# xcmyz/FastVocoder

Measured on AMD Instinct MI355X. Metric: audio samples/sec + RTF @22.05kHz, HiFi-GAN-light, 1/2/4/8 MI355X, higher is better.
Workload: dtype f32 (products as split-f16 pairs, fp32 accumulate); 1 GPU; HiFi-GAN light (conf/hifigan/light.yaml) generator forward, mel 80x1000, batch 1 utterance(s) per GPU, 240000 samples each; BASELINE.json configs[1]; global_batch=1, frames=1000, parallelism=single GPU, plan_ops_per_forward=25

## Files before the change

### fastvocoder_amd/_native.py

```python
import ctypes
import os
import subprocess

import torch

_HERE = os.path.dirname(os.path.abspath(__file__))
LIB_PATH = os.path.join(_HERE, "libfastvocoder_hip.so")
_CSRC = os.path.join(_HERE, "csrc")
SOURCES = ["conv_mfma.hip", "api.hip", "plan.hip", "pack.hip", "pqmf.hip", "wav_sink.hip", "mel.hip", "resample.hip", "griffin_lim.hip", "stft_loss.hip", "stft_loss_grad.hip", "stft_mag_grad.hip", "disc.hip", "disc_grad.hip", "disc_wgrad.hip", "mpd.hip", "mpd_grad.hip", "mpd_wgrad.hip", "gen_grad.hip", "gen_grad_bf16.hip", "basis_grad.hip", "basis_learn.hip", "optim.hip", "conv_inst_narrow.hip",
           "pair_launch.hip", "pair_inst_c16.hip", "pair_inst_c32.hip", "pairh_inst_c16.hip", "pairh_inst_c32.hip",
           "convh_launch.hip", "convh_inst_c64.hip", "convh_inst_c128.hip", "convt_inst.hip",
           "convg_inst.hip", "convr_inst.hip", "convtn_inst.hip", "convk_inst.hip", "convq2_inst.hip",
           "mrfh_launch.hip", "mrfh_inst_a.hip", "mrfh_inst_b.hip", "mrfw_inst.hip", "convtl_inst.hip", "convs2_inst.hip", "convu2_inst.hip"] + \
          [f"conv_inst_s{i}.hip" for i in range(6)]
HEADERS = ["fv_internal.h", "launch_host.hpp", "conv_kernels.hpp", "pair_kernels.hpp", "pair_inst.hpp", "pairh_kernels.hpp",
           "pairh_inst.hpp", "convh_kernels.hpp", "convh_inst.hpp", "convr_kernels.hpp",
           "convtn_kernels.hpp", "convk_kernels.hpp", "convq2_kernels.hpp", "mrfh_kernels.hpp", "mrfh_inst.hpp", "mrfw_kernels.hpp", "convtl_kernels.hpp", "convs2_kernels.hpp", "convu2_kernels.hpp", "api_internal.h", "stft_core.hpp", "basis_grad_host.hpp", "wgrad_tile.hpp", "gen_grad_host.hpp"]

PAD_ZERO, PAD_REFLECT = 0, 1
PAD_CAUSAL = 2
POST_NONE, POST_TANH, POST_RELU = 0, 1, 2
SLOT_NONE, SLOT_IN, SLOT_OUT, SLOT_TMP0, MAX_SLOTS = -1, 0, 1, 2, 32
SLOT_AUX_IN0, SLOT_AUX_IN1, SLOT_OUT2 = 28, 29, 30
ABI_VERSION = 18
# ... 280 lines not shown
    L.fv_pack_pair_weight.argtypes = [vp, vp, i, i, vp]
    L.fv_resblock1_fused.argtypes = [i, pp, pp, pp, pp, pp, pp, pp, ctypes.POINTER(i), i, i, i, i, f, f, vp]
    L.fv_mrf_stage.argtypes = [pp, pp, pp, pp, pp, vp, vp, ctypes.POINTER(i), i, i, i, i, f, f, i, f, vp]
    L.fv_plan_add_resblock_pair.argtypes = [vp, i, i, i, vp, vp, vp, vp, i, i, i, f, f]
    L.fv_packed_pair_floats_ex.argtypes = [i, i, i]
    L.fv_packed_pair_floats_ex.restype = i64
    L.fv_pack_pair_weight_ex.argtypes = [vp, vp, i, i, i, vp, vp]
    L.fv_resblock1_fused_ex.argtypes = [i, pp, pp, pp, pp, pp, pp, pp, pp, pp, pp, ctypes.POINTER(i), i, i, i, i, f, f,
                                        i, f, i, vp, vp]
    L.fv_plan_add_resblock_pair_ex.argtypes = [vp, i, i, i, i, i, i, vp, vp, vp, vp, i, i, i, f, f, i, f, i]
    L.fv_conv1d_split_f16.argtypes = [i, pp, pp, pp, pp, pp, pp, pp, pp, ctypes.POINTER(i), i, i, i, i, i, f, f, i, f, vp, vp]
    L.fv_plan_set_pair_output_conv.argtypes = [vp, vp, vp, i, f, i]
    L.fv_packed_mrf_stage_floats.argtypes = [i, ctypes.POINTER(i)]
    L.fv_packed_mrf_stage_floats.restype = i64
    L.fv_pack_mrf_stage_split_f16.argtypes = [pp, pp, pp, pp, vp, i, ctypes.POINTER(i), vp, vp]
    L.fv_mrf_stage_workspace_bytes.argtypes = [i]
    L.fv_mrf_stage_workspace_bytes.restype = i64
    L.fv_mrf_stage_split_f16.argtypes = [vp, vp, vp, vp, i, i, i, ctypes.POINTER(i), ctypes.POINTER(i), f, f, i, f, vp, vp, vp,
                                         vp, i64, vp, vp]
    L.fv_plan_add_mrf_stage_split_f16.argtypes = [vp, i, i, i, vp, i, ctypes.POINTER(i), ctypes.POINTER(i), f, f, i, f, vp, i64]
    L.fv_plan_add_conv1d_split_f16.argtypes = [vp, i, i, i, i, i, i, vp, vp, i, i, i, i, f, f, i, f]
    L.fv_plan_add_mrf_sum.argtypes = [vp, ctypes.POINTER(i), i, i, pp, pp, pp, pp, i, ctypes.POINTER(i), i, f, f, i, f]
    L.fv_plan_create.argtypes = [i]
    L.fv_plan_create.restype = vp
    L.fv_plan_destroy.argtypes = [vp]
    L.fv_plan_destroy.restype = None
    L.fv_plan_add_conv1d.argtypes = [vp, i, i, i, i, i, i, vp, vp, i, i, i, i, i, i, f, f, i, f]
    L.fv_plan_add_conv_transpose1d.argtypes = [vp, i, i, i, vp, vp, i, i, i, i, i, i, f, i, f]
    L.fv_plan_add_pqmf_synthesis.argtypes = [vp, i, i, vp, i, i]
    L.fv_plan_set_guard.argtypes = [vp, vp]
    L.fv_plan_check_range.argtypes = [vp, vp]
    L.fv_tuning_set.argtypes = [ctypes.c_char_p, i]
    L.fv_debug_pair_schedule.argtypes = [i, ctypes.POINTER(i), ctypes.POINTER(i), i, i, i, ctypes.POINTER(ctypes.c_uint)]
    L.fv_debug_mrf_class_schedule.argtypes = [i, i, i, i, ctypes.POINTER(ctypes.c_int64), ctypes.POINTER(ctypes.c_uint)]
    L.fv_debug_mrf_stage_class_f16.argtypes = [vp, vp, vp, i, i, i, i, ctypes.POINTER(i), ctypes.POINTER(i), f, vp, i64, vp]
    L.fv_mrf_stage_classes_f16.argtypes = [vp, vp, vp, vp, i, i, i, ctypes.POINTER(i), ctypes.POINTER(i), f, vp, i64, vp, vp]
    L.fv_plan_add_mrf_stage_classes_f16.argtypes = [vp, i, i, i, vp, i, ctypes.POINTER(i), ctypes.POINTER(i), f, vp, i64]
    L.fv_plan_set_group.argtypes = [vp, i]
    L.fv_plan_output_shape.argtypes = [vp, i, ctypes.POINTER(i), ctypes.POINTER(i64)]
    L.fv_plan_workspace_bytes.argtypes = [vp, i, i]
    L.fv_plan_workspace_bytes.restype = i64
    L.fv_plan_run.argtypes = [vp, i, i, vp, vp, vp, i64, vp]
    L.fv_plan_run_aux.argtypes = [vp, i, i, vp, vp, vp, ctypes.POINTER(vp), ctypes.POINTER(i), vp, i64, vp]
    L.fv_plan_set_output_offset.argtypes = [vp, i, i]
    L.fv_plan_slot_shape.argtypes = [vp, i, i, ctypes.POINTER(i), ctypes.POINTER(i64)]
    L.fv_plan_num_ops.argtypes = [vp]
    L.fv_profile_enable.argtypes = [i]
    L.fv_profile_bracket_cost.argtypes = [vp, i, ctypes.POINTER(ctypes.c_double)]
    L.fv_profile_mfma_f16_rate.argtypes = [vp, i64, i, i, vp, ctypes.POINTER(ctypes.c_double)]
    L.fv_profile_collect.argtypes = [i, ctypes.POINTER(i64), ctypes.POINTER(ctypes.c_double),
                                     ctypes.POINTER(ctypes.c_double), ctypes.POINTER(ctypes.c_double)]
    if L.fv_version() != ABI_VERSION:
        raise NativeError(f"ABI mismatch: library reports {L.fv_version()}, binding expects {ABI_VERSION}")
    _lib = L
    return L


def check(rc):
    if rc != 0:
        raise NativeError(f"libfastvocoder_hip error {rc}: {lib().fv_last_error().decode()}")


def _ptr(t, name="tensor", allow_none=False):
    if t is None:
        if allow_none:
            return None
# ... 33 lines not shown
        self.t = torch.zeros(2, dtype=torch.int32).pin_memory()

    def ptr(self, i=0):
        return self.t.data_ptr() + 4 * i

    def peek(self, i=0):
        return int(self.t[i])

    def clear(self, i=0):
        self.t[i] = 0


def tuning_set(key, value):
    check(lib().fv_tuning_set(key.encode(), int(value)))


def debug_pair_schedule(n_items, cost, nblk, mode=0, three_members=False):
    n = len(n_items)
    arr = ctypes.c_int * n
    table = (ctypes.c_uint * 512)()
    rc = lib().fv_debug_pair_schedule(n, arr(*[int(v) for v in n_items]), arr(*[int(v) for v in cost]), int(nblk), int(mode),
                                      1 if three_members else 0, table)
    check(rc if rc < 0 else 0)
    if rc == 1:
        out = []
        for b in range(nblk):
            w0, w1 = table[2 * b], table[2 * b + 1]
            e = [w0 & 0xFFFF, w0 >> 16, w1 & 0xFFFF]
            out.append([(v & 2047, v >> 11) for v in e[:n]])
        return 1, out
    if rc == 2:
        return 2, [int(table[i]) for i in range(nblk)]
    return 0, None


def mrf_class_schedule(batch, t, nblk, force=False):
    info = (ctypes.c_int64 * 12)()
    table = (ctypes.c_uint * 512)()
    check(lib().fv_debug_mrf_class_schedule(int(batch), int(t), int(nblk), 1 if force else 0, info, table))
    keys = ("split", "n_a", "n_b", "makespan", "makespan_one", "reach_a", "reach_b", "window", "cost_a", "cost_b", "cost_one")
    out = {k: int(info[i]) for i, k in enumerate(keys)}
    out["split"] = bool(out["split"])
    out["ranges"] = [(int(table[2 * i]), int(table[2 * i + 1])) for i in range(out["n_a"] + out["n_b"])]
    return out


def _flag_ptr(flag):
    if flag is None:
        return None
    if isinstance(flag, GuardWord):
        return flag.ptr(1)
    if isinstance(flag, int):
        return flag
    return flag.data_ptr()


def _guard_ptr(guard):
    if guard is None:
        return None
    if isinstance(guard, GuardWord):
        return guard.ptr(0)
    return guard.data_ptr()



def fold_weight_norm(v, g):
# ... 1624 lines not shown
```

### fastvocoder_amd/csrc/api.hip

```cpp
#include <stdarg.h>
#include <stdio.h>
#include <stdlib.h>

#include <string>
#include <mutex>
#include <utility>
#include <vector>

#include <ctype.h>
#include <string.h>
#include <unistd.h>

#include "api_internal.h"
#include "launch_host.hpp"

namespace fv {

static thread_local std::string g_err;

int fail(int code, const char* fmt, ...) {
    char buf[512];
    va_list ap;
    va_start(ap, fmt);
    vsnprintf(buf, sizeof(buf), fmt, ap);
// ... 276 lines not shown
namespace fv {
int allow_dynamic_lds(const void* kernel, size_t bytes) {
    if (bytes <= 64 * 1024) return 0;
    struct Grant { const void* kernel; int device; size_t bytes; };
    static std::mutex mu;
    static std::vector<Grant> granted;
    int dev = 0;
    FV_HIP(hipGetDevice(&dev));
    std::lock_guard<std::mutex> lock(mu);
    for (Grant& g : granted)
        if (g.kernel == kernel && g.device == dev) {
            if (g.bytes >= bytes) return 0;
            FV_HIP(hipFuncSetAttribute(kernel, hipFuncAttributeMaxDynamicSharedMemorySize, (int)bytes));
            g.bytes = bytes;
            return 0;
        }
    FV_HIP(hipFuncSetAttribute(kernel, hipFuncAttributeMaxDynamicSharedMemorySize, (int)bytes));
    granted.push_back({kernel, dev, bytes});
    return 0;
}

static Tuning g_tuning;
static std::once_flag g_tuning_once;
struct TuningEntry {
    const char* key;
    int Tuning::*field;
};
static const TuningEntry kTuningTable[] = {
    {"pair_dbg", &Tuning::pair_dbg},       {"dbg", &Tuning::conv_dbg},           {"sched", &Tuning::sched},
    {"sched_switch", &Tuning::sched_switch}, {"convh_skel", &Tuning::convh_skel}, {"convp_skel", &Tuning::convp_skel},
    {"convq_skel", &Tuning::convq_skel},   {"pair128_unfused", &Tuning::pair128_unfused},
    {"convg_rows64", &Tuning::convg_rows64}, {"stack_items", &Tuning::stack_items}, {"stack_wide", &Tuning::stack_wide},
    {"convp_wide", &Tuning::convp_wide},   {"convq_wide", &Tuning::convq_wide},
    {"convh_rows64", &Tuning::convh_rows64},  {"convt_rows64", &Tuning::convt_rows64},
    {"pairh_skel", &Tuning::pairh_skel},   {"pair_skel", &Tuning::pair_skel},    {"convh_blocks", &Tuning::convh_blocks},
    {"pair_blocks", &Tuning::pair_blocks}, {"sum3_min", &Tuning::sum3_min},      {"lds_budget", &Tuning::lds_budget},
    {"units", &Tuning::units},             {"shape16", &Tuning::shape16},        {"shape32", &Tuning::shape32},
    {"shape64", &Tuning::shape64},         {"krows", &Tuning::krows},            {"grid_cap", &Tuning::grid_cap},
    {"no_group", &Tuning::no_group},       {"mrf_blocks", &Tuning::mrf_blocks},  {"mrf_shape", &Tuning::mrf_shape},
    {"mrf_prio", &Tuning::mrf_prio},       {"convt_lean", &Tuning::convt_lean},
    {"mrf_cost_a", &Tuning::mrf_cost_a},   {"mrf_cost_b", &Tuning::mrf_cost_b},  {"mrf_cost_one", &Tuning::mrf_cost_one},
    {"convs_ringfree", &Tuning::convs_ringfree}, {"convu_resident", &Tuning::convu_resident},
};
static void tuning_from_env() {
    const char* on = getenv("FV_TUNING");
    if (!on || atoi(on) != 1) return;
    for (const TuningEntry& e : kTuningTable) {
        char name[64] = "FV_";
        size_t n = 3;
        for (const char* c = e.key; *c && n + 1 < sizeof(name); ++c) name[n++] = (char)toupper((unsigned char)*c);
        name[n] = 0;
        const char* v = getenv(name);
        if (v && *v) g_tuning.*(e.field) = atoi(v);
    }
    const char* tp = getenv("FV_PAIR_TRACE_PTR");
    if (tp && *tp) g_tuning.trace_ptr = strtoull(tp, nullptr, 0);
}
const Tuning& tuning() {
    std::call_once(g_tuning_once, tuning_from_env);
    return g_tuning;
}

int device_cu_count() {
    static int cus = 0;
    if (!cus) {
        int dev = 0, v = 0;
// ... 885 lines not shown
        if (strcmp(e.key, key) == 0) {
            g_tuning.*(e.field) = value;
            return 0;
        }
    static const char* const kRetiredKeys[] = {"convp_pp"};
    for (const char* retired : kRetiredKeys)
        if (value == 0 && strcmp(retired, key) == 0) return 0;
    return fail(FV_ERR_INVALID_ARG, "tuning_set: unknown key '%s'", key);
}

int fv_debug_pair_schedule(int n_members, const int* n_items, const int* cost, int nblk, int mode, int three_members,
                           unsigned* table) {
    if (!n_items || !cost || !table) return fail(FV_ERR_INVALID_ARG, "debug_pair_schedule: null argument");
    if (n_members < 1 || n_members > 3) return fail(FV_ERR_INVALID_ARG, "debug_pair_schedule: %d members", n_members);
    if (mode != 0 && mode != 1) return fail(FV_ERR_INVALID_ARG, "debug_pair_schedule: mode %d", mode);
    if (nblk < 1 || nblk > (mode == 0 ? fv::kSchedBlocks : 2 * fv::kSchedBlocks))
        return fail(FV_ERR_INVALID_ARG, "debug_pair_schedule: %d blocks", nblk);
    fv::PairParams p = {};
    p.n_members = n_members;
    long long n[3] = {0, 0, 0};
    for (int m = 0; m < n_members; ++m) {
        if (n_items[m] < 0 || n_items[m] >= (1LL << 31) / nblk || cost[m] < 1 || cost[m] > 65535)
            return fail(FV_ERR_INVALID_ARG, "debug_pair_schedule: member %d", m);
        p.m[m].n_items = n_items[m];
        p.m[m].cost = cost[m];
        n[m] = n_items[m];
    }
    if (mode == 0) fv::pair_schedule(p, nblk, three_members != 0);
    else fv::pair_cut_schedule(p, nblk, n);
    memcpy(table, p.sched, sizeof(p.sched));
    return p.sched_on;
}

int fv_profile_enable(int on) {
    g_prof_on = on != 0;
    g_prof_need_start = true;
    return 0;
}

__global__ void profile_null_kernel() {}

int fv_profile_bracket_cost(void* stream, int n, double* ms_per_bracket) {
    if (n <= 0 || !ms_per_bracket) return fail(FV_ERR_INVALID_ARG, "profile_bracket_cost: n=%d", n);
    hipStream_t s = (hipStream_t)stream;
    ScopedEvents events((size_t)n + 4);
    if (int rc = events.create()) return rc;
    const std::vector<hipEvent_t>& ev = events.ev;
    for (int i = 0; i < 8; ++i) hipLaunchKernelGGL(profile_null_kernel, dim3(1), dim3(64), 0, s);
    FV_HIP(hipEventRecord(ev[n], s));
    for (int i = 0; i < n; ++i) {
        hipLaunchKernelGGL(profile_null_kernel, dim3(1), dim3(64), 0, s);
        FV_HIP(hipEventRecord(ev[i], s));
    }
    FV_HIP(hipEventRecord(ev[n + 1], s));
    for (int i = 0; i < n; ++i) hipLaunchKernelGGL(profile_null_kernel, dim3(1), dim3(64), 0, s);
    FV_HIP(hipEventRecord(ev[n + 2], s));
    FV_HIP(hipEventSynchronize(ev[n + 2]));
    float with = 0.f, without = 0.f;
    FV_HIP(hipEventElapsedTime(&with, ev[n], ev[n - 1]));
    FV_HIP(hipEventElapsedTime(&without, ev[n + 1], ev[n + 2]));
    const double cost = ((double)with - (double)without) / n;
    *ms_per_bracket = cost > 0 ? cost : 0;
    return 0;
}

typedef _Float16 peak_f16x8 __attribute__((ext_vector_type(8)));
// ... 76 lines not shown
```

### fastvocoder_amd/csrc/convh_launch.hip

```cpp
#include <stdlib.h>
#include <string.h>

#include <algorithm>
#include <array>
#include <map>
#include <mutex>
#include <vector>

#include "launch_host.hpp"

namespace fv {

extern template int launch_convh_geom<4, 2>(const PairParams&, int, size_t, hipStream_t);
extern template int launch_convh_geom<2, 2>(const PairParams&, int, size_t, hipStream_t);


void pair_schedule(PairParams& p, int nblk, bool three_members) {
    typedef std::array<unsigned, 2 * kSchedBlocks> Table;
    static std::mutex mu;
    static std::map<std::array<int, 9>, Table> cache;
    p.sched_on = 0;
    const Tuning& tn = tuning();
    if (tn.sched == 0) return;
    long long items = 0;
// ... 250 lines not shown
    if (p.B <= 0 || p.T <= 0) return 0;
    if (C != 128 && C != 256 && C != 512)
        return fail(FV_ERR_UNSUPPORTED, "split-f16 two-source 1x1 conv: C = %d (128, 256 or 512)", C);
    if (int rc = check_desc_range(fam, C, p.T)) return rc;
    if (int rc = check_slopes(fam, p.slope, p.act_slope)) return rc;
    PairMember& mb = p.m[0];
    if (int rc = check_tensors(fam, mb, -1, kNeedX2 | kNeedY)) return rc;
    if (int rc = check_aligned(fam, mb, 0)) return rc;
    p.n_members = 1;
    p.ctot = C;
    p.nch = 2 * C / 128;
    p.nmt = C / 64;
    p.reflect = 0;
    p.out_div = 1.f;
    const int NTC = 128;
    mb.k = 1;
    mb.n_tiles = (p.T + NTC - 1) / NTC;
    const bool wide = tuning().convg_rows64 < 0 ? (long long)mb.n_tiles * p.B * (p.nmt / 2) * 10 >= 7LL * device_cu_count()
                                                : !tuning().convg_rows64;
    mb.n_items = mb.n_tiles * p.B * (wide ? p.nmt / 2 : p.nmt);
    mb.cost = 1;
    LdsLayout lds;
    p.x_off = lds.add(4 * 16384 / 4);
    p.img_off = lds.add(4 * 128 * 128 / 4);
    p.nblk = (int)persistent_blocks(mb.n_items, 1, tuning().convh_blocks);
    p.sched_on = 0;
    set_debug(p);
    ProfileScope prof(s, FV_KERNEL_CONVG, Work{2.0 * p.B * (double)C * 2 * C * p.T,
                                               4.0 * (2.0 * C * C + (double)p.B * C * p.T * (3 + (mb.res ? 1 : 0) + (mb.y_act ? 1 : 0)))});
    return wide ? launch_convr_geom(p, lds.bytes(), s) : launch_convg_geom(p, lds.bytes(), s);
}

constexpr int kPair64Wide = 65, kPair128Wide = 129;
template <int DIL, int C>
int launch_convq2_dil(const PairParams& p, size_t lds, hipStream_t s);
extern template int launch_convq2_dil<1, 128>(const PairParams&, size_t, hipStream_t);
extern template int launch_convq2_dil<3, 128>(const PairParams&, size_t, hipStream_t);
extern template int launch_convq2_dil<5, 128>(const PairParams&, size_t, hipStream_t);
extern template int launch_convq2_dil<1, 64>(const PairParams&, size_t, hipStream_t);
extern template int launch_convq2_dil<3, 64>(const PairParams&, size_t, hipStream_t);
extern template int launch_convq2_dil<5, 64>(const PairParams&, size_t, hipStream_t);
extern template int launch_convq2_dil<1, kPair64Wide>(const PairParams&, size_t, hipStream_t);
extern template int launch_convq2_dil<3, kPair64Wide>(const PairParams&, size_t, hipStream_t);
extern template int launch_convq2_dil<5, kPair64Wide>(const PairParams&, size_t, hipStream_t);
extern template int launch_convq2_dil<1, kPair128Wide>(const PairParams&, size_t, hipStream_t);
extern template int launch_convq2_dil<3, kPair128Wide>(const PairParams&, size_t, hipStream_t);

#ifndef FV_WARM_TILES
#define FV_WARM_TILES 1
#endif
static void warm_run_costs(PairParams& p, long long items, int nm) {
    if (!FV_WARM_TILES || items < 8LL * p.nblk) return;
    for (int i = 0; i < p.n_members; ++i) p.m[i].cost *= nm - (p.m[i].k - 1);
}

struct FusedPair {
    int C;
    int narrow, wide;
    int Tuning::*wide_from;
    int wide_dil;
    int Tuning::*skel;
    int skel_auto;
    bool three_members;
    int kind;
};
static const FusedPair kFusedPair64 = {64, 128, 256, &Tuning::convp_wide, 5, &Tuning::convp_skel, 0, false, FV_KERNEL_CONVH64};
static const FusedPair kFusedPair128 = {128, 64, 128, &Tuning::convq_wide, 3, &Tuning::convq_skel, 5, true, FV_KERNEL_CONVH128};

static int launch_fused_pair(const FusedPair& f, PairParams& p, int dil, hipStream_t s) {
    const char* const fam = "resblock pair";
    const int C = f.C;
    if (p.B <= 0 || p.T <= 0) return 0;
    if (dil != 1 && dil != 3 && dil != 5) return fail(FV_ERR_UNSUPPORTED, "resblock pair: dilation %d (1, 3 or 5)", dil);
    if (int rc = check_launch(fam, p, C)) return rc;
    sort_members_by_taps(p);
    long long wide_items = 0;
    for (int i = 0; i < p.n_members; ++i) wide_items += (long long)p.B * ((p.T + f.wide - p.m[i].k) / (f.wide + 1 - p.m[i].k));
    const bool wide = dil <= f.wide_dil && wide_items * 10 >= (long long)(tuning().*f.wide_from) * device_cu_count();
    const int NM = wide ? f.wide : f.narrow;
    const int skel = f.skel_auto && tuning().*f.skel < 0 ? f.skel_auto : tuning().*f.skel;
    int img_bytes = 0;
    long long items = 0;
    for (int i = 0; i < p.n_members; ++i) {
        PairMember& mb = p.m[i];
        if (int rc = check_taps(fam, mb.k)) return rc;
        if (int rc = check_member(fam, mb, i, kNeedW2 | kNeedY)) return rc;
        const int nout = NM - (mb.k - 1);
        mb.n_tiles = (p.T + nout - 1) / nout;
        mb.n_items = mb.n_tiles * p.B;
        mb.cost = C / 32 * mb.k + skel;
        const int xrows = (NM + (mb.k - 1) * dil + 3) / 4 * 4;
        const int img = 4 * C * ((xrows + 15) / 16 * 16);
        if (img > img_bytes) img_bytes = img;
        items += mb.n_items;
    }
    LdsLayout lds;
    p.x_off = 0;
    p.img_off = lds.add((size_t)img_bytes / 4);
    p.mid_off = lds.add((size_t)4 * C * (NM + 16) / 4);
    p.bias_off = lds.add(4 * (size_t)C + 16);
    if (int rc = check_lds(fam, lds.bytes())) return rc;
    p.nblk = (int)persistent_blocks(items, 1, tuning().convh_blocks);
    pair_schedule(p, p.nblk, f.three_members);
    if (!p.sched_on) {
        warm_run_costs(p, items, NM);
        cut_table(p, p.nblk);
    }
    set_debug(p);
    ProfileScope prof(s, f.kind, pair_work(p, C));
    const size_t bytes = lds.bytes();
    if (C == 64)
        return wide ? by_dilation<1, 3, 5>(dil, [&](auto d) { return launch_convq2_dil<decltype(d)::value, kPair64Wide>(p, bytes, s); })
                    : by_dilation<1, 3, 5>(dil, [&](auto d) { return launch_convq2_dil<decltype(d)::value, 64>(p, bytes, s); });
    return wide ? by_dilation<1, 3, 3>(dil, [&](auto d) { return launch_convq2_dil<decltype(d)::value, kPair128Wide>(p, bytes, s); })
                : by_dilation<1, 3, 5>(dil, [&](auto d) { return launch_convq2_dil<decltype(d)::value, 128>(p, bytes, s); });
}

int launch_convp(PairParams p, int dil, hipStream_t s) { return launch_fused_pair(kFusedPair64, p, dil, s); }
int launch_convq(PairParams p, int dil, hipStream_t s) { return launch_fused_pair(kFusedPair128, p, dil, s); }

}
```

### fastvocoder_amd/csrc/convq2_inst.hip

```cpp
#include "convq2_kernels.hpp"
namespace fv {
template <int DIL, int C>
int launch_convq2_dil(const PairParams& p, size_t lds, hipStream_t s) {
    if (int rc = allow_dynamic_lds(reinterpret_cast<const void*>(convq2_kernel<DIL, C>), lds)) return rc;
    hipLaunchKernelGGL((convq2_kernel<DIL, C>), dim3(p.nblk), dim3(512), lds, s, p);
    FV_HIP(hipGetLastError());
    return 0;
}
template int launch_convq2_dil<1, 128>(const PairParams&, size_t, hipStream_t);
template int launch_convq2_dil<3, 128>(const PairParams&, size_t, hipStream_t);
template int launch_convq2_dil<5, 128>(const PairParams&, size_t, hipStream_t);
template int launch_convq2_dil<1, 64>(const PairParams&, size_t, hipStream_t);
template int launch_convq2_dil<3, 64>(const PairParams&, size_t, hipStream_t);
template int launch_convq2_dil<5, 64>(const PairParams&, size_t, hipStream_t);
template int launch_convq2_dil<1, kPair64Wide>(const PairParams&, size_t, hipStream_t);
template int launch_convq2_dil<3, kPair64Wide>(const PairParams&, size_t, hipStream_t);
template int launch_convq2_dil<5, kPair64Wide>(const PairParams&, size_t, hipStream_t);
template int launch_convq2_dil<1, kPair128Wide>(const PairParams&, size_t, hipStream_t);
template int launch_convq2_dil<3, kPair128Wide>(const PairParams&, size_t, hipStream_t);
}
```

### fastvocoder_amd/csrc/convq2_kernels.hpp

```cpp
#pragma once
#include "convh_kernels.hpp"
#ifndef FV_WARM_TILES
#define FV_WARM_TILES 1
#endif

namespace fv {

template <int KT_, int DIL_>
struct ConvQGeom {
    static constexpr int KT = KT_, DIL = DIL_, C = 128, CG = 4, CB = 16, NFW = 2, NT = 512;
    static constexpr int NM = 64;
    static constexpr int NOUT = NM - (KT - 1);
    static constexpr int P1 = (KT - 1) * DIL / 2, P2 = (KT - 1) / 2;
    static constexpr int NSTEP = KT * CG;
    static constexpr int NST = 2 * NSTEP;
    static constexpr int XROWS = (NM + (KT - 1) * DIL + 3) / 4 * 4;
    static constexpr int XRP = (XROWS + 15) / 16 * 16;
    static constexpr int XHALF = CB * XRP * 16;
    static constexpr int XR = (XROWS * CB + NT - 1) / NT, XRM = XR;
    static constexpr int MRP = NM + 16;
    static constexpr int MHALF = CB * MRP * 16;
    static constexpr int STAGE_BYTES = 16384, RING = 3, AHEAD = RING - 1;
    static constexpr int WTILE = NSTEP * 8192;
    static constexpr int RAWST = NST - 8;
#ifndef FV_CONVQ_BDEPTH
#define FV_CONVQ_BDEPTH 2
#endif
    static constexpr int BD = FV_CONVQ_BDEPTH;
    static constexpr int NRAW = XRM * 8;
    static_assert(KT - 1 <= 16 && NSTEP >= 8, "taps");
    static_assert(((CG - 1) * 4 * XRP + (KT - 1) * DIL + 16 * (NFW - 1)) * 16 + 16 < 65536, "ds_read immediate range");
};

template <int KT_, int DIL_>
struct ConvPGeom {
    typedef ConvHGeom<2, 2, KT_, DIL_> H;
    static constexpr int KT = KT_, DIL = DIL_, C = 64, NFW = 2;
    static constexpr int NM = H::NTC;
    static constexpr int NOUT = NM - (KT - 1);
    static constexpr int P1 = (KT - 1) * DIL / 2, P2 = (KT - 1) / 2;
    static constexpr int NST1 = H::NST, NST = 2 * NST1;
    static constexpr int NUNIT1 = H::NUNIT;
    static constexpr int MRP = NM + 16;
    static constexpr int MHALF = (C / 8) * MRP * 16;
    static constexpr int RAWST = NST - 4, RESST = NST - 2;
    static constexpr int NRAW = H::NRAW, NRES = 8 * NFW;
    static_assert(KT - 1 <= 16 && NST1 >= 3, "taps");
};


constexpr int kPair64Wide = 65;
constexpr int kPair128Wide = 129;
template <int KT_, int DIL_, int C_>
struct ConvQ2Geom;
template <int KT_, int DIL_>
struct ConvQ2Geom<KT_, DIL_, 128> : ConvQGeom<KT_, DIL_> {
    typedef ConvQGeom<KT_, DIL_> IMG;
    static constexpr int WN = 1;
    static constexpr int WBYTES = 2 * IMG::WTILE;
};
template <int KT_, int DIL_>
struct ConvQ2Geom<KT_, DIL_, 64> : ConvPGeom<KT_, DIL_> {
    typedef typename ConvPGeom<KT_, DIL_>::H IMG;
    static constexpr int WN = 2;
    static constexpr int CG = 2, CB = 8, NT = 512;
    static constexpr int NSTEP = IMG::NSTEP, XRP = IMG::XRP, XHALF = IMG::XHALF, WTILE = IMG::WTILE, NRAW = IMG::NRAW;
    static constexpr int WBYTES = IMG::WTILE;
};
template <int KT_, int DIL_>
struct ConvWideImg {
    static constexpr int C = 64, CB = 8, NT = 512;
    static constexpr int XROWS = (256 + (KT_ - 1) * DIL_ + 3) / 4 * 4;
    static constexpr int XRP = (XROWS + 15) / 16 * 16;
    static constexpr int XHALF = CB * XRP * 16;
    static constexpr int XR = (XROWS * CB + NT - 1) / NT;
    static constexpr int NRAW = XR * 8;
};
template <int KT_, int DIL_>
struct ConvQ2Geom<KT_, DIL_, kPair64Wide> {
    typedef ConvWideImg<KT_, DIL_> IMG;
    static constexpr int KT = KT_, DIL = DIL_, C = 64, CG = 2, CB = 8, NT = 512, WN = 4;
    static constexpr int NM = 256, NOUT = NM - (KT - 1);
    static constexpr int P1 = (KT - 1) * DIL / 2, P2 = (KT - 1) / 2;
    static constexpr int NSTEP = KT * CG;
    static constexpr int XRP = IMG::XRP, XHALF = IMG::XHALF, NRAW = IMG::NRAW;
    static constexpr int MRP = NM + 16, MHALF = CB * MRP * 16;
    static constexpr int WTILE = NSTEP * 8192, WBYTES = WTILE;
    static_assert(((CG - 1) * 4 * XRP + (KT - 1) * DIL + 16 * 3) * 16 + 16 < 65536, "ds_read immediate range");
};
template <int KT_, int DIL_>
struct ConvWideImg128 {
    static constexpr int C = 128, CB = 16, NT = 512;
    static constexpr int XROWS = (128 + (KT_ - 1) * DIL_ + 3) / 4 * 4;
    static constexpr int XRP = (XROWS + 15) / 16 * 16;
    static constexpr int XHALF = CB * XRP * 16;
    static constexpr int XR = (XROWS * CB + NT - 1) / NT;
    static constexpr int NRAW = XR * 8;
};
template <int KT_, int DIL_>
struct ConvQ2Geom<KT_, DIL_, kPair128Wide> {
    typedef ConvWideImg128<KT_, DIL_> IMG;
    static constexpr int KT = KT_, DIL = DIL_, C = 128, CG = 4, CB = 16, NT = 512, WN = 2;
    static constexpr int NM = 128, NOUT = NM - (KT - 1);
    static constexpr int P1 = (KT - 1) * DIL / 2, P2 = (KT - 1) / 2;
    static constexpr int NSTEP = KT * CG;
    static constexpr int XRP = IMG::XRP, XHALF = IMG::XHALF, NRAW = IMG::NRAW;
    static constexpr int MRP = NM + 16, MHALF = CB * MRP * 16;
    static constexpr int WTILE = NSTEP * 8192, WBYTES = 2 * WTILE;
    static_assert(((CG - 1) * 4 * XRP + (KT - 1) * DIL + 16 * 3) * 16 + 16 < 65536, "ds_read immediate range");
    static_assert(2 * XHALF + 2 * MHALF + (4 * C + 16) * 4 <= 160 * 1024, "LDS: dilation 1 and 3 only");
};
#ifndef FV_Q2_ILV
#define FV_Q2_ILV 1
#endif
template <int KT_, int DIL_, int C_>
struct ConvQ2Run : ConvQ2Geom<KT_, DIL_, C_> {
    typedef ConvQ2Geom<KT_, DIL_, C_> B;
    static constexpr int NFW = 4;
    static constexpr int NH = C_ == kPair64Wide || C_ == kPair128Wide ? 2 : 1;
    static constexpr int NSLAB = B::C / (16 * NH);
#ifndef FV_Q2_DEEP
#define FV_Q2_DEEP 1
#endif
    static constexpr int QD = NH == 2 ? 1 : !FV_Q2_DEEP || B::C == 128 ? 3 : KT_ == 3 ? 5 : KT_ == 7 ? 6 : 3;
    static constexpr int NA = 2 * NH;
    static constexpr bool ILV = FV_Q2_ILV && NH == 1;
    static constexpr int NSEQ = 2 * B::NSTEP;
    static constexpr bool RES_EARLY = NH == 1;
    static constexpr int NRES = 4 * NFW * NH;
    static constexpr int RAWK = NSEQ - QD;
    static_assert(NSEQ % (QD + 1) == 0, "the A queue runs on from tile to tile: slot = K step % (QD + 1)");
    static_assert(B::NM == 64 * B::WN && NSLAB * B::WN == 8, "8 waves: row slabs x column groups of 64");
};

template <class G>
__device__ __forceinline__ void convq2_run_member(const PairParams& p, const PairMember& mb, int item0, int hi_item,
                                                  float* smem, int wave, int lane_in, bool first) {
    typedef __attribute__((address_space(3))) const f16x8 LdsH8;
    int lane = lane_in;
    asm volatile("" : "+v"(lane));
    const int tid = wave * 64 + lane;
    char* const ximg = reinterpret_cast<char*>(smem + p.img_off);
    char* const mimg = reinterpret_cast<char*>(smem + p.mid_off);
    float* const bl = smem + p.bias_off;
    const int n = lane & 15, kb = lane >> 4;
    const int ws = wave % G::NSLAB;
    const int col0 = (wave / G::NSLAB) * 64 + n;
    const char* const bptr = ximg + (kb * G::XRP + col0) * 16;
    const char* const mptr = mimg + (kb * G::MRP + col0) * 16;
    const int row0 = 16 * G::NH * ws + 4 * kb;
    char* const mw = mimg + ((2 * G::NH * ws + (kb >> 1)) * G::MRP + col0) * 16 + 8 * (kb & 1);

    const size_t ustride = (size_t)G::C * (size_t)p.T;
    const unsigned ubytes = (unsigned)G::C * (unsigned)p.T * 4u;
    const unsigned t4 = (unsigned)p.T * 4u;
    const __amdgpu_buffer_rsrc_t rw1 = make_rsrc(mb.w1, (unsigned)G::WBYTES);
    const __amdgpu_buffer_rsrc_t rw2 = make_rsrc(mb.w2, (unsigned)G::WBYTES);
    const int s16 = G::NH * ws;
    const unsigned aoff = (unsigned)((s16 >> 2) * G::WTILE + (s16 & 3) * 2048 + lane * 16);
    auto load_a = [&](auto SC, f16x8 (&dst)[G::NH][2]) {
        constexpr int S = decltype(SC)::value % G::NSEQ;
        constexpr int step = S % G::NSTEP;
#pragma unroll
        for (int h = 0; h < G::NH; ++h)
#pragma unroll
// ... 309 lines not shown
```

### fastvocoder_amd/csrc/fv_internal.h

```cpp
#pragma once
#include <hip/hip_runtime.h>

#include <vector>
#include <stdint.h>

#include "../../include/fastvocoder_hip.h"

namespace fv {

int fail(int code, const char* fmt, ...);

#define FV_HIP(call)                                                              \
    do {                                                                          \
        hipError_t e_ = (call);                                                   \
        if (e_ != hipSuccess)                                                     \
            return ::fv::fail((int)e_, "%s failed: %s", #call, hipGetErrorString(e_)); \
    } while (0)

static inline int round_up(int v, int m) { return (v + m - 1) / m * m; }

int check_conv_args(int Cin, int Cout, int k, int dil);
int check_convt_split_args(int Cin, int Cout, int k, int stride, int pad, int out_pad);

static inline int pad_rows(int M) { return M <= 16 ? 16 : round_up(M, 32); }
// ... 65 lines not shown
    int dbg;
    double alg_flops;
};

struct GroupParams {
    ConvParams p[3];
    int grid_x[3];
};

struct Sum3Params {
    ConvParams p[3];
    int xbuf_max, wbuf_max;
};
int launch_conv_sum3(ConvParams* ps, hipStream_t stream);

int allow_dynamic_lds(const void* kernel, size_t bytes);
int device_cu_count();
struct Tuning {
    int pair_dbg = 0;
    int conv_dbg = 0;
    int sched = 1;
    int sched_switch = 4;
    int convh_skel = -1;
    int convp_skel = 5;
    int convq_skel = -1;
    int pair128_unfused = 0;
    int convh_rows64 = -1;
    int convt_rows64 = -1;
    int convs_ringfree = -1;
    int convu_resident = 1;
    int convt_lean = 50;
    int convq_wide = 20;
    int convp_wide = 20;
    int stack_wide = 10;
    int stack_items = 1 << 20;
    int convg_rows64 = -1;
    int pairh_skel = -1;
    int pair_skel = -1;
    int convh_blocks = 0;
    int pair_blocks = 0;
    int mrf_blocks = 0;
    int mrf_shape = 0;
    int mrf_cost_a = 585;
    int mrf_cost_b = 661;
    int mrf_cost_one = 1490;
    int mrf_prio = 1;
    int sum3_min = 800;
    int lds_budget = 39;
    int units = 500;
    int shape16 = -1, shape32 = -1, shape64 = -1;
    int krows = 176;
    int grid_cap = 1024;
    int no_group = 0;
    unsigned long long trace_ptr = 0;
};
const Tuning& tuning();

struct PairMember {
    const float* x;
    const float* x2;
    const float* w1;
    const float* w2;
    const float* b1;
    const float* b2;
    float* y;
    float* y_act;
// ... 45 lines not shown
struct PairShape {
    int MH, NF, NG;
    int NW, NM;
    int XS, NXI, MS;
    int WF;
    int NOUT;
};
PairShape pair_shape(int C, int k, int dil);
#ifndef FV_PAIRH32_NG
#define FV_PAIRH32_NG 15
#endif
#ifndef FV_PAIRH16_NF
#define FV_PAIRH16_NF 2
#define FV_PAIRH16_NG 8
#endif
struct PairHShape {
    int MH, NF, NG, NM;
    int KS;
    int XROWS, WB;
    int MROWS;
    int XIMG, MIMG;
    int NOUT;
};
PairHShape pairh_shape(int C, int k, int dil);
struct ConvHShape {
    int CG, NFW, NTC;
    int NSTEP, NST;
    int XROWS, XIMG, NMT;
    int NCH;
};
ConvHShape convh_shape(int C, int k, int dil);
int launch_convh(PairParams p, int C, int dil, hipStream_t stream);
void pair_schedule(PairParams& p, int nblk, bool three_members = false);
void pair_cut_schedule(PairParams& p, int nblk, const long long* n);
int launch_convp(PairParams p, int dil, hipStream_t stream);
int launch_convq(PairParams p, int dil, hipStream_t stream);
template <int CG, int NFW>
int launch_convh_geom(const PairParams& p, int dil, size_t lds, hipStream_t s);
int launch_convt(PairParams p, int Cin, int Cout, int stride, int pad, int Tout, hipStream_t stream);
int launch_convt_geom(const PairParams& p, int cg, size_t lds, hipStream_t s);
int launch_convs2_geom(const PairParams& p, int dil, int nh, size_t lds, hipStream_t s);
int launch_convu2_geom(const PairParams& p, int nch, hipStream_t s);
int launch_convtl_geom(const PairParams& p, int cg, hipStream_t s);
inline bool convtn_shape(int Cin, int Cout, int k, int stride) { return Cin == 32 && Cout == 16 && k == 4 && stride == 2; }
constexpr int kTnPackedFloats = 2048 + 32;
int launch_convtn(const PairParams& p, int Tout, hipStream_t s);
int launch_pack_convtn(const float* w, float* packed, const float* inv, int* range_flag, hipStream_t s);
inline bool convk_shape(int C, int k, int dil) { return (C == 32 || C == 64 || C == 128 || C == 256) && k == 3 && (dil == 1 || dil == 3 || dil == 9); }
inline int convk_tile_columns(int C) { return C == 256 ? 32 : 256 / (C / 32); }
int launch_convk(const PairParams& p, int C, int dil, hipStream_t s);
inline bool mpd_period_ok(int p) { return p == 2 || p == 3 || p == 5 || p == 7 || p == 11; }
inline int64_t period_conv_rows(int64_t H) { return (H - 1) / 3 + 1; }
struct MpdView {
    int64_t n_pad, H, H1;
};
inline MpdView mpd_view(int64_t T, int period) {
    const int64_t n_pad = T % period ? period - T % period : 0;
    const int64_t H = (T + n_pad) / period;
    return MpdView{n_pad, H, period_conv_rows(H)};
}
int launch_pack_convk(const float* w1, const float* w2, const float* ws, float* packed, int C, int* range_flag, hipStream_t s);
int launch_convg(PairParams p, int C, hipStream_t stream);
int launch_convg_geom(const PairParams& p, size_t lds, hipStream_t s);
int launch_convr_geom(const PairParams& p, size_t lds, hipStream_t s);
int launch_convs_geom(const PairParams& p, int dil, size_t lds, hipStream_t s);
int launch_convu_geom(const PairParams& p, size_t lds, hipStream_t s);
// ... 161 lines not shown
```

### include/fastvocoder_hip.h

```cpp
#ifndef FASTVOCODER_HIP_H
#define FASTVOCODER_HIP_H

#include <stddef.h>
#include <stdint.h>

#ifdef __cplusplus
extern "C" {
#endif

#define FV_ABI_VERSION 18

#define FV_ERR_INVALID_ARG (-1)
#define FV_ERR_UNSUPPORTED (-2)
#define FV_ERR_WORKSPACE (-3)
#define FV_ERR_RANGE (-4)
#define FV_ERR_RANGE_LOW (-5)
#define FV_GUARD_HIGH 0x001
#define FV_GUARD_LOW 0x100

#define FV_PAD_ZERO 0
#define FV_PAD_REFLECT 1
#define FV_PAD_CAUSAL 2

#define FV_POST_NONE 0
// ... 378 lines not shown
int fv_plan_add_conv_post_pqmf(fv_plan_t* plan, int x_slot, int y_slot, const float* packed, const float* bias, int Cin,
                               int S, int k, int pad, float pre_slope, int post, const float* h, int ntaps);

int fv_plan_set_output_offset(fv_plan_t* plan, int aux_slot, int y2_slot);

int fv_plan_set_sum_order(fv_plan_t* plan, int own_first);

int fv_plan_set_group(fv_plan_t* plan, int group);

int fv_plan_output_shape(fv_plan_t* plan, int T, int* out_channels, int64_t* out_len);
int fv_plan_slot_shape(fv_plan_t* plan, int T, int slot, int* channels, int64_t* len);
int64_t fv_plan_workspace_bytes(fv_plan_t* plan, int B, int T);

int fv_plan_run(fv_plan_t* plan, int B, int T, const float* in, float* out,
                void* workspace, int64_t workspace_bytes, void* stream);

int fv_plan_run_aux(fv_plan_t* plan, int B, int T, const float* in, float* out, float* out2,
                    const float* const* aux_in, const int* aux_batched, void* workspace,
                    int64_t workspace_bytes, void* stream);

int fv_generator_run(fv_plan_t* plan, int B, int T, const float* mel, float* out, void* workspace,
                     int64_t workspace_bytes, void* stream);

int fv_div_probe(unsigned first_bits, int64_t n, float d, unsigned long long* mismatches, void* stream);

int fv_plan_num_ops(fv_plan_t* plan);

int fv_plan_set_guard(fv_plan_t* plan, int* word);
int fv_plan_check_range(fv_plan_t* plan, void* stream);

int fv_tuning_set(const char* key, int value);
int fv_debug_pair_schedule(int n_members, const int* n_items, const int* cost, int nblk, int mode, int three_members,
                           unsigned* table);
int fv_debug_mrf_class_schedule(int B, int T, int nblk, int force, int64_t* info, unsigned* table);
int fv_debug_mrf_stage_class_f16(const float* x, const float* packed, float* y, int cls, int B, int C, int T, const int* k,
                                 const int* dil, float slope, void* workspace, int64_t workspace_bytes, void* stream);

#define FV_KERNEL_CONV_MFMA32 0
#define FV_KERNEL_CONV_MFMA16 1
#define FV_KERNEL_CONV_NARROW 2
#define FV_KERNEL_PAIR16 3
#define FV_KERNEL_PAIR32 4
#define FV_KERNEL_PAIRH16 5
#define FV_KERNEL_PAIRH32 6
#define FV_KERNEL_CONVH64 7
#define FV_KERNEL_CONVH128 8
#define FV_KERNEL_CONVT 9
#define FV_KERNEL_CONVG 10
#define FV_KERNEL_STACK 11
#define FV_KERNEL_MRF16 12
#define FV_KERNEL_MRF32 13
int fv_profile_enable(int on);
int fv_profile_bracket_cost(void* stream, int n, double* ms_per_bracket);
int fv_profile_mfma_f16_rate(float* scratch, long long scratch_floats, int launches, int iters, void* stream, double* tflops);
int fv_profile_collect(int kind, int64_t* launches, double* ms, double* flops, double* bytes);

#ifdef __cplusplus
}
#endif
#endif
```

Measured before the change: 412.9 million samples/s.

## Pick 80-column tiles for 11-tap resblock members by schedule makespan

Adds an 80-column tile variant of the 128-channel fused resblock pair kernel for the 11-tap member. By default a cached planner simulates the persistent-block schedule at widths 64 and 80 and keeps whichever has the smaller makespan. Wider tiles cut the halo recompute that 11 taps cost on 64-column tiles, and the warm-run cost model is rescaled for mixed widths. In exchange it adds three new kernel instantiations, extra LDS use and a host-side planning step, plus a debug API to inspect the chosen plan.

```diff
diff --git a/fastvocoder_amd/_native.py b/fastvocoder_amd/_native.py
--- a/fastvocoder_amd/_native.py
+++ b/fastvocoder_amd/_native.py
@@ -336,6 +336,7 @@
     L.fv_plan_check_range.argtypes = [vp, vp]
     L.fv_tuning_set.argtypes = [ctypes.c_char_p, i]
     L.fv_debug_pair_schedule.argtypes = [i, ctypes.POINTER(i), ctypes.POINTER(i), i, i, i, ctypes.POINTER(ctypes.c_uint)]
+    L.fv_debug_pair_widths.argtypes = [i, i, i, i, i, ctypes.POINTER(i), i, ctypes.POINTER(ctypes.c_int64)]
     L.fv_debug_mrf_class_schedule.argtypes = [i, i, i, i, ctypes.POINTER(ctypes.c_int64), ctypes.POINTER(ctypes.c_uint)]
     L.fv_debug_mrf_stage_class_f16.argtypes = [vp, vp, vp, i, i, i, i, ctypes.POINTER(i), ctypes.POINTER(i), f, vp, i64, vp]
     L.fv_mrf_stage_classes_f16.argtypes = [vp, vp, vp, vp, i, i, i, ctypes.POINTER(i), ctypes.POINTER(i), f, vp, i64, vp, vp]
@@ -435,6 +436,15 @@
     if rc == 2:
         return 2, [int(table[i]) for i in range(nblk)]
     return 0, None
+
+
+def debug_pair_widths(channels, batch, t, dil, taps, blocks):
+    n = len(taps)
+    info = (ctypes.c_int64 * 12)()
+    check(lib().fv_debug_pair_widths(int(channels), int(batch), int(t), int(dil), n, (ctypes.c_int * n)(*[int(k) for k in taps]),
+                                     int(blocks), info))
+    return {"widths": [int(info[m]) for m in range(n)], "items": [int(info[3 + m]) for m in range(n)],
+            "costs": [int(info[6 + m]) for m in range(n)], "makespan": int(info[9]), "nblk": int(info[10])}
 
 
 def mrf_class_schedule(batch, t, nblk, force=False):
diff --git a/fastvocoder_amd/csrc/api.hip b/fastvocoder_amd/csrc/api.hip
--- a/fastvocoder_amd/csrc/api.hip
+++ b/fastvocoder_amd/csrc/api.hip
@@ -332,6 +332,7 @@
     {"convq_skel", &Tuning::convq_skel},   {"pair128_unfused", &Tuning::pair128_unfused},
     {"convg_rows64", &Tuning::convg_rows64}, {"stack_items", &Tuning::stack_items}, {"stack_wide", &Tuning::stack_wide},
     {"convp_wide", &Tuning::convp_wide},   {"convq_wide", &Tuning::convq_wide},
+    {"convq_nm11", &Tuning::convq_nm11},   {"convq_cost80", &Tuning::convq_cost80},
     {"convh_rows64", &Tuning::convh_rows64},  {"convt_rows64", &Tuning::convt_rows64},
     {"pairh_skel", &Tuning::pairh_skel},   {"pair_skel", &Tuning::pair_skel},    {"convh_blocks", &Tuning::convh_blocks},
     {"pair_blocks", &Tuning::pair_blocks}, {"sum3_min", &Tuning::sum3_min},      {"lds_budget", &Tuning::lds_budget},
@@ -1283,6 +1284,28 @@
     return p.sched_on;
 }
 
+int fv_debug_pair_widths(int C, int B, int T, int dil, int n_members, const int* taps, int blocks, int64_t* info) {
+    if (!taps || !info) return fail(FV_ERR_INVALID_ARG, "debug_pair_widths: null argument");
+    if (C != 128) return fail(FV_ERR_UNSUPPORTED, "debug_pair_widths: C = %d (128: the other launchers have one width)", C);
+    if (dil != 1 && dil != 3 && dil != 5) return fail(FV_ERR_UNSUPPORTED, "debug_pair_widths: dilation %d (1, 3 or 5)", dil);
+    if (n_members < 1 || n_members > 3) return fail(FV_ERR_INVALID_ARG, "debug_pair_widths: %d members", n_members);
+    if (B < 1 || T < 1 || blocks < 1 || (double)B * T >= 2147483647.0)
+        return fail(FV_ERR_INVALID_ARG, "debug_pair_widths: B=%d T=%d on %d blocks (B x T < 2^31)", B, T, blocks);
+    for (int m = 0; m < n_members; ++m)
+        if ((taps[m] != 3 && taps[m] != 7 && taps[m] != 11) || (m > 0 && taps[m] > taps[m - 1]))
+            return fail(FV_ERR_INVALID_ARG, "debug_pair_widths: member %d: %d taps (3, 7 or 11, largest first)", m, taps[m]);
+    const fv::PairWidthPlan pl = fv::pair_width_plan(B, T, n_members, taps, blocks);
+    for (int m = 0; m < 3; ++m) {
+        info[m] = m < n_members ? pl.nm[m] : 0;
+        info[3 + m] = m < n_members ? pl.n_items[m] : 0;
+        info[6 + m] = m < n_members ? pl.cost[m] : 0;
+    }
+    info[9] = pl.makespan;
+    info[10] = pl.nblk;
+    info[11] = 0;
+    return 0;
+}
+
 int fv_profile_enable(int on) {
     g_prof_on = on != 0;
     g_prof_need_start = true;
diff --git a/fastvocoder_amd/csrc/convh_launch.hip b/fastvocoder_amd/csrc/convh_launch.hip
--- a/fastvocoder_amd/csrc/convh_launch.hip
+++ b/fastvocoder_amd/csrc/convh_launch.hip
@@ -306,6 +306,7 @@
 }
 
 constexpr int kPair64Wide = 65, kPair128Wide = 129;
+constexpr int kPair128Col80 = 130;
 template <int DIL, int C>
 int launch_convq2_dil(const PairParams& p, size_t lds, hipStream_t s);
 extern template int launch_convq2_dil<1, 128>(const PairParams&, size_t, hipStream_t);
@@ -319,13 +320,16 @@
 extern template int launch_convq2_dil<5, kPair64Wide>(const PairParams&, size_t, hipStream_t);
 extern template int launch_convq2_dil<1, kPair128Wide>(const PairParams&, size_t, hipStream_t);
 extern template int launch_convq2_dil<3, kPair128Wide>(const PairParams&, size_t, hipStream_t);
+extern template int launch_convq2_dil<1, kPair128Col80>(const PairParams&, size_t, hipStream_t);
+extern template int launch_convq2_dil<3, kPair128Col80>(const PairParams&, size_t, hipStream_t);
+extern template int launch_convq2_dil<5, kPair128Col80>(const PairParams&, size_t, hipStream_t);
 
 #ifndef FV_WARM_TILES
 #define FV_WARM_TILES 1
 #endif
-static void warm_run_costs(PairParams& p, long long items, int nm) {
+static void warm_run_costs(PairParams& p, long long items, const int* nm, bool mixed) {
     if (!FV_WARM_TILES || items < 8LL * p.nblk) return;
-    for (int i = 0; i < p.n_members; ++i) p.m[i].cost *= nm - (p.m[i].k - 1);
+    for (int i = 0; i < p.n_members; ++i) p.m[i].cost *= (nm[i] - (p.m[i].k - 1)) * (mixed ? 320 / nm[i] : 1);
 }
 
 struct FusedPair {
@@ -341,6 +345,65 @@
 static const FusedPair kFusedPair64 = {64, 128, 256, &Tuning::convp_wide, 5, &Tuning::convp_skel, 0, false, FV_KERNEL_CONVH64};
 static const FusedPair kFusedPair128 = {128, 64, 128, &Tuning::convq_wide, 3, &Tuning::convq_skel, 5, true, FV_KERNEL_CONVH128};
 
+static int fused_pair_skel(const FusedPair& f) { return f.skel_auto && tuning().*f.skel < 0 ? f.skel_auto : tuning().*f.skel; }
+
+static PairWidthPlan pair_width_candidate(int B, int T, int n_members, const int* taps, int blocks, int nm11) {
+    const Tuning& tn = tuning();
+    PairWidthPlan pl = {};
+    PairParams p = {};
+    p.n_members = n_members;
+    long long items = 0;
+    for (int m = 0; m < n_members; ++m) {
+        const int nm = taps[m] == 11 ? nm11 : 64, nout = nm - (taps[m] - 1);
+        pl.nm[m] = nm;
+        pl.n_tiles[m] = (T + nout - 1) / nout;
+        pl.n_items[m] = pl.n_tiles[m] * B;
+        pl.cost[m] = nm == 80 && tn.convq_cost80 > 0 ? tn.convq_cost80 : 128 / 32 * taps[m] * nm / 64 + fused_pair_skel(kFusedPair128);
+        p.m[m].n_items = pl.n_items[m];
+        p.m[m].cost = pl.cost[m];
+        items += pl.n_items[m];
+    }
+    pl.nblk = (int)std::min<long long>(blocks, items);
+    pl.makespan = -1;
+    pair_schedule(p, pl.nblk, kFusedPair128.three_members);
+    if (p.sched_on != 1) return pl;
+    for (int b = 0; b < pl.nblk; ++b) {
+        const int cnt[3] = {(int)((p.sched[2 * b] >> 11) & 31u), (int)(p.sched[2 * b] >> 27), (int)((p.sched[2 * b + 1] >> 11) & 31u)};
+        long long load = 0;
+        for (int m = 0; m < n_members; ++m)
+            if (cnt[m]) load += (long long)cnt[m] * pl.cost[m] + (load > 0 ? tn.sched_switch : 0);
+        pl.makespan = std::max(pl.makespan, load);
+    }
+    return pl;
+}
+
+PairWidthPlan pair_width_plan(int B, int T, int n_members, const int* taps, int blocks) {
+    const Tuning& tn = tuning();
+    typedef std::array<int, 13> Key;
+    static std::mutex mu;
+    static std::map<Key, PairWidthPlan> cache;
+    Key key = {B, T, n_members, 0, 0, 0, blocks, tn.convq_nm11, tn.convq_cost80, fused_pair_skel(kFusedPair128), tn.sched, tn.sched_switch, 0};
+    bool has11 = false;
+    for (int m = 0; m < n_members; ++m) {
+        key[3 + m] = taps[m];
+        has11 = has11 || taps[m] == 11;
+    }
+    {
+        std::lock_guard<std::mutex> lock(mu);
+        auto it = cache.find(key);
+        if (it != cache.end()) return it->second;
+    }
+    PairWidthPlan pl = pair_width_candidate(B, T, n_members, taps, blocks, has11 && tn.convq_nm11 == 80 ? 80 : 64);
+    if (has11 && tn.convq_nm11 != 64 && tn.convq_nm11 != 80 && pl.makespan >= 0) {
+        const PairWidthPlan w = pair_width_candidate(B, T, n_members, taps, blocks, 80);
+        if (w.makespan >= 0 && w.makespan < pl.makespan) pl = w;
+    }
+    std::lock_guard<std::mutex> lock(mu);
+    if (cache.size() >= 512) cache.clear();
+    cache.emplace(key, pl);
+    return pl;
+}
+
 static int launch_fused_pair(const FusedPair& f, PairParams& p, int dil, hipStream_t s) {
     const char* const fam = "resblock pair";
     const int C = f.C;
@@ -351,33 +414,49 @@
     long long wide_items = 0;
     for (int i = 0; i < p.n_members; ++i) wide_items += (long long)p.B * ((p.T + f.wide - p.m[i].k) / (f.wide + 1 - p.m[i].k));
     const bool wide = dil <= f.wide_dil && wide_items * 10 >= (long long)(tuning().*f.wide_from) * device_cu_count();
-    const int NM = wide ? f.wide : f.narrow;
-    const int skel = f.skel_auto && tuning().*f.skel < 0 ? f.skel_auto : tuning().*f.skel;
-    int img_bytes = 0;
+    const int skel = fused_pair_skel(f);
+    for (int i = 0; i < p.n_members; ++i)
+        if (int rc = check_taps(fam, p.m[i].k)) return rc;
+    int nm[3], cost[3];
+    for (int i = 0; i < p.n_members; ++i) {
+        nm[i] = wide ? f.wide : f.narrow;
+        cost[i] = C / 32 * p.m[i].k + skel;
+    }
+    if (C == 128 && !wide) {
+        int taps[3] = {0, 0, 0};
+        for (int i = 0; i < p.n_members; ++i) taps[i] = p.m[i].k;
+        const PairWidthPlan pl = pair_width_plan(p.B, p.T, p.n_members, taps, (int)persistent_blocks(1LL << 40, 1, tuning().convh_blocks));
+        for (int i = 0; i < p.n_members; ++i) {
+            nm[i] = pl.nm[i];
+            cost[i] = pl.cost[i];
+        }
+    }
+    const bool col80 = nm[0] == 80;
+    int img_bytes = 0, nm_max = 0;
     long long items = 0;
     for (int i = 0; i < p.n_members; ++i) {
         PairMember& mb = p.m[i];
-        if (int rc = check_taps(fam, mb.k)) return rc;
         if (int rc = check_member(fam, mb, i, kNeedW2 | kNeedY)) return rc;
-        const int nout = NM - (mb.k - 1);
+        const int nout = nm[i] - (mb.k - 1);
         mb.n_tiles = (p.T + nout - 1) / nout;
         mb.n_items = mb.n_tiles * p.B;
-        mb.cost = C / 32 * mb.k + skel;
-        const int xrows = (NM + (mb.k - 1) * dil + 3) / 4 * 4;
+        mb.cost = cost[i];
+        const int xrows = (nm[i] + (mb.k - 1) * dil + 3) / 4 * 4;
         const int img = 4 * C * ((xrows + 15) / 16 * 16);
         if (img > img_bytes) img_bytes = img;
+        if (nm[i] > nm_max) nm_max = nm[i];
         items += mb.n_items;
     }
     LdsLayout lds;
     p.x_off = 0;
     p.img_off = lds.add((size_t)img_bytes / 4);
-    p.mid_off = lds.add((size_t)4 * C * (NM + 16) / 4);
+    p.mid_off = lds.add((size_t)4 * C * (nm_max + 16) / 4);
     p.bias_off = lds.add(4 * (size_t)C + 16);
     if (int rc = check_lds(fam, lds.bytes())) return rc;
     p.nblk = (int)persistent_blocks(items, 1, tuning().convh_blocks);
     pair_schedule(p, p.nblk, f.three_members);
     if (!p.sched_on) {
-        warm_run_costs(p, items, NM);
+        warm_run_costs(p, items, nm, col80);
         cut_table(p, p.nblk);
     }
     set_debug(p);
@@ -386,6 +465,7 @@
     if (C == 64)
         return wide ? by_dilation<1, 3, 5>(dil, [&](auto d) { return launch_convq2_dil<decltype(d)::value, kPair64Wide>(p, bytes, s); })
                     : by_dilation<1, 3, 5>(dil, [&](auto d) { return launch_convq2_dil<decltype(d)::value, 64>(p, bytes, s); });
+    if (col80) return by_dilation<1, 3, 5>(dil, [&](auto d) { return launch_convq2_dil<decltype(d)::value, kPair128Col80>(p, bytes, s); });
     return wide ? by_dilation<1, 3, 3>(dil, [&](auto d) { return launch_convq2_dil<decltype(d)::value, kPair128Wide>(p, bytes, s); })
                 : by_dilation<1, 3, 5>(dil, [&](auto d) { return launch_convq2_dil<decltype(d)::value, 128>(p, bytes, s); });
 }
diff --git a/fastvocoder_amd/csrc/convq2_inst.hip b/fastvocoder_amd/csrc/convq2_inst.hip
--- a/fastvocoder_amd/csrc/convq2_inst.hip
+++ b/fastvocoder_amd/csrc/convq2_inst.hip
@@ -18,4 +18,7 @@
 template int launch_convq2_dil<5, kPair64Wide>(const PairParams&, size_t, hipStream_t);
 template int launch_convq2_dil<1, kPair128Wide>(const PairParams&, size_t, hipStream_t);
 template int launch_convq2_dil<3, kPair128Wide>(const PairParams&, size_t, hipStream_t);
+template int launch_convq2_dil<1, kPair128Col80>(const PairParams&, size_t, hipStream_t);
+template int launch_convq2_dil<3, kPair128Col80>(const PairParams&, size_t, hipStream_t);
+template int launch_convq2_dil<5, kPair128Col80>(const PairParams&, size_t, hipStream_t);
 }
diff --git a/fastvocoder_amd/csrc/convq2_kernels.hpp b/fastvocoder_amd/csrc/convq2_kernels.hpp
--- a/fastvocoder_amd/csrc/convq2_kernels.hpp
+++ b/fastvocoder_amd/csrc/convq2_kernels.hpp
@@ -6,10 +6,10 @@
 
 namespace fv {
 
-template <int KT_, int DIL_>
+template <int KT_, int DIL_, int NF_ = 4>
 struct ConvQGeom {
     static constexpr int KT = KT_, DIL = DIL_, C = 128, CG = 4, CB = 16, NFW = 2, NT = 512;
-    static constexpr int NM = 64;
+    static constexpr int NM = 16 * NF_;
     static constexpr int NOUT = NM - (KT - 1);
     static constexpr int P1 = (KT - 1) * DIL / 2, P2 = (KT - 1) / 2;
     static constexpr int NSTEP = KT * CG;
@@ -29,7 +29,8 @@
     static constexpr int BD = FV_CONVQ_BDEPTH;
     static constexpr int NRAW = XRM * 8;
     static_assert(KT - 1 <= 16 && NSTEP >= 8, "taps");
-    static_assert(((CG - 1) * 4 * XRP + (KT - 1) * DIL + 16 * (NFW - 1)) * 16 + 16 < 65536, "ds_read immediate range");
+    static_assert(((CG - 1) * 4 * XRP + (KT - 1) * DIL + 16 * (NF_ - 1)) * 16 + 16 < 65536, "ds_read immediate range");
+    static_assert(2 * XHALF + 2 * MHALF + (4 * C + 16) * 4 <= 160 * 1024, "LDS");
 };
 
 template <int KT_, int DIL_>
@@ -51,6 +52,7 @@
 
 constexpr int kPair64Wide = 65;
 constexpr int kPair128Wide = 129;
+constexpr int kPair128Col80 = 130;
 template <int KT_, int DIL_, int C_>
 struct ConvQ2Geom;
 template <int KT_, int DIL_>
@@ -110,13 +112,21 @@
     static_assert(((CG - 1) * 4 * XRP + (KT - 1) * DIL + 16 * 3) * 16 + 16 < 65536, "ds_read immediate range");
     static_assert(2 * XHALF + 2 * MHALF + (4 * C + 16) * 4 <= 160 * 1024, "LDS: dilation 1 and 3 only");
 };
+template <int KT_, int DIL_>
+struct ConvQ2Geom<KT_, DIL_, kPair128Col80> : ConvQ2Geom<KT_, DIL_, 128> {};
+template <int DIL_>
+struct ConvQ2Geom<11, DIL_, kPair128Col80> : ConvQGeom<11, DIL_, 5> {
+    typedef ConvQGeom<11, DIL_, 5> IMG;
+    static constexpr int WN = 1;
+    static constexpr int WBYTES = 2 * IMG::WTILE;
+};
 #ifndef FV_Q2_ILV
 #define FV_Q2_ILV 1
 #endif
 template <int KT_, int DIL_, int C_>
 struct ConvQ2Run : ConvQ2Geom<KT_, DIL_, C_> {
     typedef ConvQ2Geom<KT_, DIL_, C_> B;
-    static constexpr int NFW = 4;
+    static constexpr int NFW = B::NM / (16 * B::WN);
     static constexpr int NH = C_ == kPair64Wide || C_ == kPair128Wide ? 2 : 1;
     static constexpr int NSLAB = B::C / (16 * NH);
 #ifndef FV_Q2_DEEP
@@ -130,7 +140,8 @@
     static constexpr int NRES = 4 * NFW * NH;
     static constexpr int RAWK = NSEQ - QD;
     static_assert(NSEQ % (QD + 1) == 0, "the A queue runs on from tile to tile: slot = K step % (QD + 1)");
-    static_assert(B::NM == 64 * B::WN && NSLAB * B::WN == 8, "8 waves: row slabs x column groups of 64");
+    static_assert(B::NM == 16 * NFW * B::WN && NSLAB * B::WN == 8 && (NFW == 4 || B::WN == 1),
+                  "8 waves: row slabs x column groups of 64 (one group: of 16 NFW)");
 };
 
 template <class G>
diff --git a/fastvocoder_amd/csrc/fv_internal.h b/fastvocoder_amd/csrc/fv_internal.h
--- a/fastvocoder_amd/csrc/fv_internal.h
+++ b/fastvocoder_amd/csrc/fv_internal.h
@@ -121,6 +121,8 @@
     int convt_lean = 50;
     int convq_wide = 20;
     int convp_wide = 20;
+    int convq_nm11 = -1;
+    int convq_cost80 = -1;
     int stack_wide = 10;
     int stack_items = 1 << 20;
     int convg_rows64 = -1;
@@ -232,6 +234,12 @@
 ConvHShape convh_shape(int C, int k, int dil);
 int launch_convh(PairParams p, int C, int dil, hipStream_t stream);
 void pair_schedule(PairParams& p, int nblk, bool three_members = false);
+struct PairWidthPlan {
+    int nm[3], n_tiles[3], n_items[3], cost[3];
+    int nblk;
+    long long makespan;
+};
+PairWidthPlan pair_width_plan(int B, int T, int n_members, const int* taps, int blocks);
 void pair_cut_schedule(PairParams& p, int nblk, const long long* n);
 int launch_convp(PairParams p, int dil, hipStream_t stream);
 int launch_convq(PairParams p, int dil, hipStream_t stream);
diff --git a/include/fastvocoder_hip.h b/include/fastvocoder_hip.h
--- a/include/fastvocoder_hip.h
+++ b/include/fastvocoder_hip.h
@@ -434,6 +434,7 @@
 int fv_tuning_set(const char* key, int value);
 int fv_debug_pair_schedule(int n_members, const int* n_items, const int* cost, int nblk, int mode, int three_members,
                            unsigned* table);
+int fv_debug_pair_widths(int C, int B, int T, int dil, int n_members, const int* taps, int blocks, int64_t* info);
 int fv_debug_mrf_class_schedule(int B, int T, int nblk, int force, int64_t* info, unsigned* table);
 int fv_debug_mrf_stage_class_f16(const float* x, const float* packed, float* y, int cls, int B, int C, int T, const int* k,
                                  const int* dil, float slope, void* workspace, int64_t workspace_bytes, void* stream);
```

Result: faster. 424.0 million samples/s (median of 6 runs) (+2.7%).
